# tamask1s/rspt

Measured on NVIDIA B200. Metric: compress_raw_GBps, higher is better.
Workload: dtype u8

## Files before the change

### include/rspt_gpu.h

```cpp
#ifndef RSPT_GPU_H_
#define RSPT_GPU_H_

#include <stddef.h>
#include <stdint.h>

#ifdef __cplusplus
extern "C" {
#endif

#define RSPT_GPU_ABI_VERSION 1

enum {
    RSPT_XDELTA_HZR = 0,
    RSPT_HZR = 1,
    RSPT_HADAMARD = 2,
    RSPT_DCT = 3
};

enum {
    RSPT_OK = 0,
    RSPT_E_ARG = -1,
    RSPT_E_CUDA = -2,
    RSPT_E_CAPACITY = -3,
    RSPT_E_STREAM = -4,
// ... 57 lines not shown
int rspt_gpu_sync(rspt_gpu_packer* p);
const char* rspt_gpu_last_error(const rspt_gpu_packer* p);

typedef struct {
    uint64_t frames_compressed, frames_decompressed;
    uint64_t raw_bytes_in, compressed_bytes_out;
    uint64_t blocks_copy, blocks_huff, blocks_fill;
    uint64_t escalations;
    uint64_t crc_failures;
    uint64_t kernel_launches;
} rspt_gpu_counters;
int rspt_gpu_get_counters(rspt_gpu_packer* p, rspt_gpu_counters* out);

enum {
    RSPT_STAGE_TRANSFORM = 0,
    RSPT_STAGE_HIST = 1,
    RSPT_STAGE_TREE = 2,
    RSPT_STAGE_LAYOUT = 3,
    RSPT_STAGE_ENCODE = 4,
    RSPT_STAGE_PARSE = 5,
    RSPT_STAGE_DECODE = 6,
    RSPT_STAGE_INVERSE = 7,
    RSPT_STAGE_COUNT = 8
};
int rspt_gpu_set_stage_timing(rspt_gpu_packer* p, int enable);
int rspt_gpu_get_stage_times(rspt_gpu_packer* p, double* ms ,
                             uint64_t* calls , int reset);

int rspt_gpu_debug_planes(rspt_gpu_packer* p, const uint8_t* d_src, size_t n_frames,
                          uint8_t* d_planes , uint8_t* d_header );
int rspt_gpu_debug_hzr_tables(rspt_gpu_packer* p, const uint8_t* d_block, size_t n,
                              uint32_t* d_hist , uint32_t* d_codes ,
                              uint32_t* d_info );
int rspt_gpu_crc32c(const uint8_t* d_data, size_t n, uint32_t* h_crc, void* stream);

int rspt_gpu_synth_ecg(uint8_t* d_dst, uint64_t first_frame, size_t n_frames, int bps, int ch, int ns,
                       uint64_t seed, int32_t amplitude, int32_t sigma, void* stream);

int rspt_gpu_prdn_terms(const uint8_t* d_orig, const uint8_t* d_dec, size_t n_frames, int bps, int ch,
                        int ns, double* h_out, void* stream);

int rspt_gpu_comm_unique_id(uint8_t id[128]);
int rspt_gpu_comm_init(int world, const uint8_t id[128], int rank, int device, void** comm);
int rspt_gpu_comm_destroy(void* comm);

int rspt_gpu_allgather_totals(void* comm, const uint64_t* d_total, uint64_t* d_all_totals, void* stream);

int rspt_gpu_rebase_offsets(uint64_t* d_offsets, size_t n_frames_plus_1, const uint64_t* d_all_totals,
                            int rank, void* stream);

int rspt_gpu_place_offsets_async(rspt_gpu_packer* p, void* comm, uint64_t* d_offsets, size_t n_frames, int rank, int world);
int rspt_gpu_place_join(rspt_gpu_packer* p);

int rspt_gpu_set_stream(rspt_gpu_packer* p, void* stream);

int rspt_gpu_set_dct_exact(rspt_gpu_packer* p, int exact);

#ifdef __cplusplus
}
#endif
#endif
```

### rspt_b200/_lib.py

```python
from __future__ import annotations

import ctypes as C
import os

HERE = os.path.dirname(os.path.abspath(__file__))
LIB_PATH = os.path.join(HERE, "librspt_gpu.so")

KINDS = {"xdelta_hzr": 0, "hzr": 1, "hadamard": 2, "dct": 3}
STAGES = ["transform", "hist", "tree", "layout", "encode", "parse", "decode", "inverse"]
ERRORS = {0: "ok", -1: "bad argument / unsupported shape", -2: "CUDA error", -3: "capacity too small",
          -4: "malformed stream", -5: "no CUDA device", -6: "CRC-32C mismatch"}

EXPORTS = [
    "rspt_gpu_create", "rspt_gpu_destroy", "rspt_gpu_frame_bytes", "rspt_gpu_header_bytes",
    "rspt_gpu_max_compressed_size", "rspt_gpu_nb", "rspt_gpu_compress_batch", "rspt_gpu_decompress_batch",
    "rspt_gpu_sidecar_bytes", "rspt_gpu_sidecar_used_bytes", "rspt_gpu_compress_host", "rspt_gpu_decompress_host",
    "rspt_gpu_compress_batch_host", "rspt_gpu_decompress_batch_host", "rspt_gpu_sync", "rspt_gpu_last_error",
    "rspt_gpu_get_counters", "rspt_gpu_debug_planes", "rspt_gpu_debug_hzr_tables", "rspt_gpu_crc32c",
    "rspt_gpu_synth_ecg", "rspt_gpu_prdn_terms", "rspt_gpu_rebase_offsets",
    "rspt_gpu_set_stage_timing", "rspt_gpu_get_stage_times", "rspt_gpu_verify_batch", "rspt_gpu_build_index",
    "rspt_gpu_prefilter_iir", "rspt_gpu_prefilter_fir",
    "rspt_gpu_ingest_create", "rspt_gpu_ingest_destroy", "rspt_gpu_ingest_next_address_to_fill", "rspt_gpu_ingest_drain",
    "rspt_gpu_comm_unique_id", "rspt_gpu_comm_init", "rspt_gpu_comm_destroy", "rspt_gpu_allgather_totals",
    "rspt_gpu_place_offsets_async", "rspt_gpu_place_join", "rspt_gpu_set_stream", "rspt_gpu_set_dct_exact",
]


class Counters(C.Structure):
    _fields_ = [(n, C.c_uint64) for n in (
        "frames_compressed", "frames_decompressed", "raw_bytes_in", "compressed_bytes_out",
        "blocks_copy", "blocks_huff", "blocks_fill", "escalations", "crc_failures", "kernel_launches")]


class RsptError(RuntimeError):
    pass


_lib = None


def lib() -> C.CDLL:
    global _lib
    if _lib is not None:
        return _lib
    if not os.path.exists(LIB_PATH):
        raise RsptError(f"{LIB_PATH} is missing: run `python -m rspt_b200.build` (nvcc, sm_100a). "
                        "There is no CPU fallback.")
    L = C.CDLL(LIB_PATH)
    sz, vp, u64 = C.c_size_t, C.c_void_p, C.c_uint64
    L.rspt_gpu_create.restype = C.c_int
    L.rspt_gpu_create.argtypes = [C.c_int, sz, sz, sz, sz, C.c_int, vp, sz, C.POINTER(vp)]
# ... 17 lines not shown
    L.rspt_gpu_prefilter_iir.argtypes = [vp, vp, sz, dp, dp, C.c_int, C.c_int]
    L.rspt_gpu_prefilter_fir.restype = C.c_int
    L.rspt_gpu_prefilter_fir.argtypes = [vp, vp, sz, dp, C.c_int]
    L.rspt_gpu_ingest_create.restype = C.c_int
    L.rspt_gpu_ingest_create.argtypes = [vp, sz, C.POINTER(vp)]
    L.rspt_gpu_ingest_destroy.restype = C.c_int
    L.rspt_gpu_ingest_destroy.argtypes = [vp]
    L.rspt_gpu_ingest_next_address_to_fill.restype = vp
    L.rspt_gpu_ingest_next_address_to_fill.argtypes = [vp]
    L.rspt_gpu_ingest_drain.restype = C.c_int
    L.rspt_gpu_ingest_drain.argtypes = [vp, C.c_int, vp, sz, vp, C.POINTER(sz)]
    L.rspt_gpu_build_index.restype = C.c_int
    L.rspt_gpu_build_index.argtypes = [vp, vp, vp, sz, vp, vp, vp]
    L.rspt_gpu_verify_batch.restype = C.c_int
    L.rspt_gpu_verify_batch.argtypes = [vp, vp, vp, sz, vp, vp]
    L.rspt_gpu_compress_host.restype = C.c_int
    L.rspt_gpu_compress_host.argtypes = [vp, vp, vp, sz, C.POINTER(sz)]
    L.rspt_gpu_decompress_host.restype = C.c_int
    L.rspt_gpu_decompress_host.argtypes = [vp, vp, C.POINTER(sz), vp]
    L.rspt_gpu_compress_batch_host.restype = C.c_int
    L.rspt_gpu_compress_batch_host.argtypes = [vp, vp, sz, vp, sz, vp]
    L.rspt_gpu_decompress_batch_host.restype = C.c_int
    L.rspt_gpu_decompress_batch_host.argtypes = [vp, vp, vp, sz, vp]
    L.rspt_gpu_sync.restype = C.c_int
    L.rspt_gpu_sync.argtypes = [vp]
    L.rspt_gpu_last_error.restype = C.c_char_p
    L.rspt_gpu_last_error.argtypes = [vp]
    L.rspt_gpu_get_counters.restype = C.c_int
    L.rspt_gpu_get_counters.argtypes = [vp, C.POINTER(Counters)]
    L.rspt_gpu_debug_planes.restype = C.c_int
    L.rspt_gpu_debug_planes.argtypes = [vp, vp, sz, vp, vp]
    L.rspt_gpu_debug_hzr_tables.restype = C.c_int
    L.rspt_gpu_debug_hzr_tables.argtypes = [vp, vp, sz, vp, vp, vp]
    L.rspt_gpu_crc32c.restype = C.c_int
    L.rspt_gpu_crc32c.argtypes = [vp, sz, C.POINTER(C.c_uint32), vp]
    L.rspt_gpu_synth_ecg.restype = C.c_int
    L.rspt_gpu_synth_ecg.argtypes = [vp, u64, sz, C.c_int, C.c_int, C.c_int, u64, C.c_int32, C.c_int32, vp]
    L.rspt_gpu_prdn_terms.restype = C.c_int
    L.rspt_gpu_prdn_terms.argtypes = [vp, vp, sz, C.c_int, C.c_int, C.c_int, C.POINTER(C.c_double), vp]
    L.rspt_gpu_rebase_offsets.restype = C.c_int
    L.rspt_gpu_rebase_offsets.argtypes = [vp, sz, vp, C.c_int, vp]
    L.rspt_gpu_set_stage_timing.restype = C.c_int
    L.rspt_gpu_set_stage_timing.argtypes = [vp, C.c_int]
    L.rspt_gpu_get_stage_times.restype = C.c_int
    L.rspt_gpu_get_stage_times.argtypes = [vp, C.POINTER(C.c_double), C.POINTER(u64), C.c_int]
    L.rspt_gpu_comm_unique_id.restype = C.c_int
    L.rspt_gpu_comm_unique_id.argtypes = [vp]
    L.rspt_gpu_comm_init.restype = C.c_int
    L.rspt_gpu_comm_init.argtypes = [C.c_int, vp, C.c_int, C.c_int, C.POINTER(vp)]
    L.rspt_gpu_comm_destroy.restype = C.c_int
    L.rspt_gpu_comm_destroy.argtypes = [vp]
    L.rspt_gpu_allgather_totals.restype = C.c_int
    L.rspt_gpu_allgather_totals.argtypes = [vp, vp, vp, vp]
    L.rspt_gpu_place_offsets_async.restype = C.c_int
    L.rspt_gpu_place_offsets_async.argtypes = [vp, vp, vp, sz, C.c_int, C.c_int]
    L.rspt_gpu_place_join.restype = C.c_int
    L.rspt_gpu_place_join.argtypes = [vp]
    L.rspt_gpu_set_stream.restype = C.c_int
    L.rspt_gpu_set_stream.argtypes = [vp, vp]
    L.rspt_gpu_set_dct_exact.restype = C.c_int
    L.rspt_gpu_set_dct_exact.argtypes = [vp, C.c_int]
    _lib = L
    return L


def check(rc: int, handle=None, what: str = "") -> None:
# ... 9 lines not shown
```

### rspt_b200/csrc/hzr_tree.cuh

```cuda
#pragma once

#include "common.cuh"

namespace rspt {

constexpr int kTreeWarps = 2;

struct TreeWarpSmem {
    uint32_t key[264];
    uint32_t icnt[260];
    uint32_t child[260];
    uint32_t ninfo[260];
    uint32_t tree[kTreeWords];
    uint16_t front[2][264];
    uint32_t pad;
};

struct Counters {
    unsigned long long frames_compressed, frames_decompressed, raw_bytes_in, compressed_bytes_out;
    unsigned long long blocks_copy, blocks_huff, blocks_fill, escalations;
    unsigned long long crc_failures;
};

__device__ __forceinline__ void blk_decode(const Shape& s, uint32_t blk, uint32_t& f, uint32_t& k, uint32_t& b)
{
    b = blk % s.nblk;
    uint32_t fk = blk / s.nblk;
    k = fk % s.nb_alloc;
    f = fk / s.nb_alloc;
}

__device__ __forceinline__ const uint8_t* blk_ptr(const uint8_t* planes, const Shape& s, uint32_t f, uint32_t k, uint32_t b)
{
    return planes + ((size_t)f * s.nb_alloc + k) * s.plane_stride + (size_t)b * kBlock;
}


__device__ __forceinline__ bool tree_prepare(TreeWarpSmem& S, const uint32_t* h, uint32_t* codes_out, uint32_t& L_out, BlkInfo& bi)
{
    const uint32_t lane = lane_id();
    uint32_t L = 0, nz = 0, nzsym = 0, zero_class = 0;
    uint32_t mykey = 0xFFFFFFFFu;
#pragma unroll
    for (int r = 0; r < 9; ++r) {
        const uint32_t sym = r * 32 + lane;
        const uint32_t c = sym < kNumSymbols ? h[sym] : 0u;
        const bool used = c != 0;
        const uint32_t m = __ballot_sync(0xFFFFFFFFu, used);
        const uint32_t pos = L + __popc(m & ((1u << lane) - 1u));
// ... 100 lines not shown
        id = take_int ? 512u + fr : li;
        wt = take_int ? ic : lc;
        lv = take_int ? ch >> 20 : 1u;
        if (take_int) {
            ic = nfr < ni ? raw & kInf : kInf;
            icf = nfr < ni ? raw & kEqNext : 0u;
        } else {
            lc = nli < L ? nk >> 9 : kInf;
        }
        fr = nfr;
        li = nli;
    };
    for (uint32_t round = 0; round + 1 < L; ++round) {
        uint32_t id0, id1, w0, w1, lv0, lv1;
        pick(id0, w0, lv0);
        pick(id1, w1, lv1);
        const uint32_t w = w0 + w1;
        if (w == last_w) {
            S.icnt[ni - 1] = w | kEqNext;
            if (ni - 1 == fr) icf = kEqNext;
        }
        if (fr == ni) {
            ic = w;
            icf = 0;
        }
        S.icnt[ni] = w;
        S.child[ni] = id0 | (id1 << 10) | ((lv0 + lv1) << 20);
        last_w = w;
        ++ni;
    }
    S.icnt[L - 2] = 0;
    S.ninfo[L - 2] = 0;
    S.front[0][0] = (uint16_t)(L - 2);
}

__device__ __forceinline__ BlkInfo tree_assign(TreeWarpSmem& S, const uint32_t L, uint32_t n, uint32_t* codes_out, uint32_t* tree_out)
{
    const uint32_t lane = lane_id();
    BlkInfo bi;
    uint32_t token_bits = 0, maxlen = 0, ntok = 0;
    {
        auto leaf = [&](uint32_t rank, uint32_t code, uint32_t depth, uint32_t off) {
            const uint32_t kv = S.key[rank];
            const uint32_t sym = 511u - (kv & 511u), cnt = kv >> 9;
            codes_out[sym] = code | (depth << 27);
            token_bits += cnt * (depth + sym_extra_bits(sym));
            ntok += cnt;
            maxlen = max(maxlen, depth);
            const unsigned long long bits = (unsigned long long)(1u | (sym << 1)) << (off & 31u);
            atomicOr(&S.tree[off >> 5], (uint32_t)bits);
            if (bits >> 32) atomicOr(&S.tree[(off >> 5) + 1], (uint32_t)(bits >> 32));
        };
        uint32_t nf = 1, cur = 0;
        const uint32_t lt = (1u << lane) - 1u;
        while (nf) {
            uint32_t nn = 0;
            for (uint32_t fb = 0; fb < nf; fb += 32) {
                const uint32_t i = fb + lane;
                const bool act = i < nf;
                uint32_t a = 0, bb = 0;
                if (act) {
                    const uint32_t j = S.front[cur][i];
                    const uint32_t ch = S.child[j], code = S.icnt[j], inf = S.ninfo[j];
                    const uint32_t depth = inf & 255u, off = inf >> 8;
                    a = ch & 1023u;
                    bb = (ch >> 10) & 1023u;
// ... 17 lines not shown
                const uint32_t ma = __ballot_sync(0xFFFFFFFFu, ia), mb = __ballot_sync(0xFFFFFFFFu, ib);
                if (ia) S.front[cur ^ 1][nn + __popc(ma & lt)] = (uint16_t)(a - 512u);
                nn += __popc(ma);
                if (ib) S.front[cur ^ 1][nn + __popc(mb & lt)] = (uint16_t)(bb - 512u);
                nn += __popc(mb);
            }
            __syncwarp();
            cur ^= 1;
            nf = nn;
        }
    }
#pragma unroll
    for (int o = 16; o > 0; o >>= 1) {
        token_bits += __shfl_xor_sync(0xFFFFFFFFu, token_bits, o);
        ntok += __shfl_xor_sync(0xFFFFFFFFu, ntok, o);
        maxlen = max(maxlen, __shfl_xor_sync(0xFFFFFFFFu, maxlen, o));
    }
    __syncwarp();
    const uint32_t tree_nbits = 11u * L - 1u;
    for (uint32_t i = lane; i < ((tree_nbits + 31u) >> 5); i += 32) tree_out[i] = S.tree[i];
    bi.tree_nbits = (uint16_t)tree_nbits;
    bi.total_bits = tree_nbits + token_bits;
    const uint32_t bytes = (bi.total_bits + 7u) >> 3;
    const bool copy = bytes > n || bytes >= kBlock || maxlen > 27u;
    bi.mode = copy ? MODE_COPY : MODE_HUFF;
    bi.payload_len = copy ? n : bytes;
    bi.fill = (uint8_t)maxlen;
    bi.n_used = (uint16_t)L;
    bi.n_tokens = (uint16_t)min(ntok, 65535u);
    return bi;
}

__device__ __forceinline__ BlkInfo warp_build_tree(TreeWarpSmem& S, const uint32_t* h, uint32_t n,
                                                   uint32_t* codes_out, uint32_t* tree_out)
{
    BlkInfo bi;
    uint32_t L;
    if (tree_prepare(S, h, codes_out, L, bi)) return bi;
    if (lane_id() == 0) tree_merge(S, L);
    __syncwarp();
    return tree_assign(S, L, n, codes_out, tree_out);
}

__device__ __forceinline__ void count_block_mode(Counters* ctr, uint32_t mode)
{
    atomicAdd(mode == MODE_FILL ? &ctr->blocks_fill : (mode == MODE_COPY ? &ctr->blocks_copy : &ctr->blocks_huff), 1ull);
}

__device__ __forceinline__ void warp_hist_from_list(const uint32_t* __restrict__ list, uint32_t m, uint32_t n, uint32_t* h)
{
    for (uint32_t i = lane_id(); i <= m; i += 32) {
        const uint32_t rs = i ? (list[i - 1] & 0xFFFFu) + 1u : 0u;
        uint32_t cur = n;
        if (i < m) {
            const uint32_t e = list[i];
            cur = e & 0xFFFFu;
            atomicAdd(&h[e >> 16], 1u);
        }
        uint32_t z = cur > rs ? cur - rs : 0u;
        while (z > kRunCap) {
            atomicAdd(&h[260], 1u);
            z -= kRunCap;
        }
        if (z) {
            const uint32_t idx = (z >= 2u) + (z >= 3u) + (z >= 7u) + (z >= 23u) + (z >= 279u);
            atomicAdd(&h[idx ? 255u + idx : 0u], 1u);
        }
    }
}

__global__ void __launch_bounds__(kTreeWarps * 32) k_hzr_tree(const uint32_t* __restrict__ hist, Shape s,
                                                               const uint8_t* __restrict__ frame_nb,
                                                               const uint8_t* __restrict__ blk_class, uint32_t cls,
                                                               uint32_t total_blocks,
                                                               uint32_t* __restrict__ codes,
                                                               uint32_t* __restrict__ tree,
                                                               BlkInfo* __restrict__ info,
                                                               Counters* __restrict__ ctr,
                                                               const uint32_t* __restrict__ list_n = nullptr, uint32_t sparse_stage = 0,
                                                               uint8_t* __restrict__ redo = nullptr,
                                                               const uint32_t* __restrict__ sub_n = nullptr,
                                                               const uint8_t* __restrict__ planes = nullptr,
                                                               uint32_t* __restrict__ lists = nullptr, uint32_t list_cap = 0)
{
    __shared__ TreeWarpSmem s_all[kTreeWarps];
    TreeWarpSmem& S = s_all[warp_id()];
    const uint32_t blk = blockIdx.x * kTreeWarps + warp_id();
    if (blk >= total_blocks) return;
    uint32_t f, k, b;
    blk_decode(s, blk, f, k, b);
    if (k >= frame_nb[f] || (blk_class && blk_class[blk] != cls)) return;
    const uint32_t n = blk_len(s, b);
    const uint32_t* h = hist + (size_t)blk * kSymStride;
    if (sub_n && list_n[blk] != kNoList) {
        const uint32_t lane = lane_id();
        const uint32_t ns = (uint32_t)s.ns, c0 = (b * kBlock) / ns, c1 = (b * kBlock + n) / ns;
        uint32_t* dst = lists + (size_t)blk * list_cap;
        uint32_t at = 0;
        for (uint32_t c = c0; c < c1; ++c) {
            const uint32_t nc = sub_n[((size_t)f * s.nb_alloc + k) * s.ch + c];
            const uint32_t* sub = reinterpret_cast<const uint32_t*>(planes + ((size_t)f * s.nb_alloc + k) * s.plane_stride + (size_t)c * ns);
            for (uint32_t i = lane; i < nc; i += 32) dst[at + i] = sub[i];
            at += nc;
        }
        uint32_t* list_hist = S.ninfo;
        static_assert(kTreeWords >= 4, "the histogram of a listed block spans ninfo[260] and tree[0..3]");
        for (uint32_t i = lane; i < (uint32_t)kSymStride; i += 32) list_hist[i] = 0;
        __syncwarp();
        warp_hist_from_list(dst, at, n, list_hist);
        __syncwarp();
        h = list_hist;
    }
    const BlkInfo bi = warp_build_tree(S, h, n, codes + (size_t)blk * kSymStride, tree + (size_t)blk * kTreeWords);
    if (lane_id() == 0) {
        info[blk] = bi;
        count_block_mode(ctr, bi.mode);
        if (redo && bi.mode != MODE_FILL && list_n[blk] != kNoList && !sparse_block_is_packed_from_list(list_n[blk], bi, sparse_stage))
            redo[f] = 1;
    }
}

__global__ void __launch_bounds__(1024) k_hzr_tree_ls(const uint32_t* __restrict__ hist, Shape s,
                                                      const uint8_t* __restrict__ frame_nb,
                                                      const uint8_t* __restrict__ blk_class, uint32_t cls,
                                                      uint32_t total_blocks,
                                                      uint32_t* __restrict__ codes,
                                                      uint32_t* __restrict__ tree,
                                                      BlkInfo* __restrict__ info,
                                                      Counters* __restrict__ ctr)
{
    extern __shared__ __align__(16) uint8_t s_tree_raw[];
    TreeWarpSmem* s_all = reinterpret_cast<TreeWarpSmem*>(s_tree_raw);
    __shared__ uint32_t s_L[32];
    const uint32_t W = blockDim.x >> 5, wid = warp_id(), lane = lane_id();
    TreeWarpSmem& S = s_all[wid];
    const uint32_t blk = blockIdx.x * W + wid;
    uint32_t f = 0, k = 0, b = 0, n = 0, L = 0;
    bool live = blk < total_blocks, merge = false;
    BlkInfo bi;
    if (live) {
        blk_decode(s, blk, f, k, b);
        live = k < frame_nb[f] && !(blk_class && blk_class[blk] != cls);
    }
    if (live) {
        n = blk_len(s, b);
        merge = !tree_prepare(S, hist + (size_t)blk * kSymStride, codes + (size_t)blk * kSymStride, L, bi);
// ... 14 lines not shown
```

### rspt_b200/csrc/packer.cuh

```cuda
#pragma once

#include <cuda_runtime.h>
#include <stdint.h>
#include <stdio.h>
#include <string.h>

#include <vector>

#include "common.cuh"
#include "hzr_encode.cuh"

struct HostPipe {
    cudaStream_t s_in, s_out;
    cudaEvent_t ev_in[2], ev_comp[2], ev_off[2], ev_out[2];
    uint8_t* d_src[2];
    uint8_t* d_dst[2];
    uint64_t* d_off[2];
    uint64_t* h_off[2];
    size_t chunk;
};

struct rspt_gpu_packer {
    rspt::Shape s;
    int device;
// ... 23 lines not shown
    uint64_t* d_all_totals;
    uint16_t* d_step_lz;
    rspt::BlkInfo* d_info;
    uint8_t* d_frame_nb;
    uint32_t* d_need;
    uint32_t* d_nb_state;
    uint32_t* d_sizes;
    uint32_t* d_blk_off;
    uint8_t* d_headers;
    int32_t* d_words;
    long long* d_sums;
    rspt::Counters* d_ctr;
    const rspt::CrcConst* d_crc;
    void* d_dec;
    uint8_t* d_dec_nb;
    int32_t* d_status_tmp;
    uint8_t* d_seg_xor;
    uint32_t segs_per_plane;
    void* d_auto_index;
    uint32_t* d_inv_tot;
    uint32_t* d_inv_flag;
    uint32_t inv_epoch;
    double* d_fir;
    size_t fir_cap;
    int32_t* d_words2;
    uint8_t* d_redo;
    uint8_t* d_redo2;
    uint32_t* d_sub_n;
    bool front_ok;
    int front_grid;
    size_t front_smem;
    uint32_t sp_stage;
    bool sparse_list;
    double2* d_twiddle;
    double2* d_post;
    float* d_cos;
    uint8_t* d_one_src;
    uint8_t* d_one_dst;
    uint64_t* d_one_off;
    uint8_t* h_pin;
    size_t h_pin_bytes;
    uint8_t* d_hb_src;
    uint8_t* d_hb_dst;
    uint64_t* d_hb_off;
    size_t hb_frames;
    HostPipe pipe;

    unsigned long long launches;
    bool timing;
    std::vector<cudaEvent_t>* ev_free;
    struct Pending { int stage; cudaEvent_t a, b; };
    std::vector<Pending>* ev_pending;
    double stage_ms[8];
    unsigned long long stage_calls[8];
    char err[256];
};

namespace rspt {

inline int fail_cuda(rspt_gpu_packer* p, cudaError_t e, const char* what)
{
    if (p) snprintf(p->err, sizeof(p->err), "CUDA error %d (%s) at %s", (int)e, cudaGetErrorString(e), what);
    return -2;
}

inline int fail_arg(rspt_gpu_packer* p, const char* what)
// ... 7 lines not shown
```

### rspt_b200/csrc/rspt_gpu.cu

```cuda
#include "../../include/rspt_gpu.h"
#include "../../include/rspt_synth.h"

#include <dlfcn.h>
#include <stdlib.h>

#include <atomic>
#include <mutex>
#include <new>
#include <vector>

#include "packer.cuh"
#include "transforms.cuh"
#include "front.cuh"
#include "hzr_decode.cuh"
#include "spectral.cuh"
#include "filters.cuh"

using namespace rspt;

namespace {

constexpr int kMaxDevices = 64;
std::mutex g_mu;
CrcConst* g_crc[kMaxDevices] = {};
// ... 368 lines not shown
    if (e == cudaSuccess && kind == RSPT_DCT) e = dct_build_tables(p);
    const size_t maxc = rspt_gpu_max_compressed_size(p);
    A(dalloc(p->d_one_src, (size_t)s.frame_bytes));
    A(dalloc(p->d_one_dst, maxc));
    A(dalloc(p->d_one_off, 2));
    p->h_pin_bytes = maxc > s.frame_bytes ? maxc : s.frame_bytes;
    p->h_pin_bytes += 64;
    if (e == cudaSuccess) e = cudaMallocHost(reinterpret_cast<void**>(&p->h_pin), p->h_pin_bytes);
    if (e == cudaSuccess) e = cudaMemsetAsync(p->d_frame_nb, (int)s.nb_init, F, p->stream);
    if (e == cudaSuccess) e = cudaMemsetAsync(p->d_ctr, 0, sizeof(Counters), p->stream);
    if (e == cudaSuccess) e = cudaMemcpyAsync(p->d_nb_state, &s.nb_init, 4, cudaMemcpyHostToDevice, p->stream);
    if (e == cudaSuccess) e = allow_smem(k_hzr_encode<2>, kEncodeSmem);
    if (e == cudaSuccess) e = allow_smem(k_hzr_encode<3>, kEncodeSmem);
    if (e == cudaSuccess) e = allow_smem(k_hzr_hist<1>, kHistSmem);
    if (e == cudaSuccess) e = allow_smem(k_hzr_hist<3>, kHistSmemList);
    if (e == cudaSuccess) e = cudaStreamCreateWithFlags(&p->side, cudaStreamNonBlocking);
    if (e == cudaSuccess) e = cudaStreamCreateWithFlags(&p->place, cudaStreamNonBlocking);
    if (e == cudaSuccess) e = cudaEventCreateWithFlags(&p->ev_place, cudaEventDisableTiming);
    for (int k = 0; k < rspt_gpu_packer::kPlaceRing && e == cudaSuccess; ++k)
        e = cudaEventCreateWithFlags(&p->ev_placed[k], cudaEventDisableTiming);
    if (e == cudaSuccess) e = cudaEventCreateWithFlags(&p->ev_fork, cudaEventDisableTiming);
    if (e == cudaSuccess) e = cudaEventCreateWithFlags(&p->ev_join, cudaEventDisableTiming);
    if (e == cudaSuccess) e = cudaEventCreateWithFlags(&p->ev_fork2, cudaEventDisableTiming);
    if (e == cudaSuccess) e = cudaEventCreateWithFlags(&p->ev_join2, cudaEventDisableTiming);
    if (e == cudaSuccess) e = allow_smem(k_hzr_encode_sparse<true>, kSparseSmem);
    if (e == cudaSuccess) e = allow_smem(k_hzr_encode_sparse<false>, kSparseSmem);
    if (e == cudaSuccess) e = front_setup(p);
    {
        const char* ev = getenv("RSPT_SPARSE_STAGE_BYTES");
        const long v = ev ? atol(ev) : (long)kSpStageBytes;
        p->sp_stage = (uint32_t)(v < 1 ? 1 : (v > (long)kSpStageBytes ? (long)kSpStageBytes : v));
        const char* el = getenv("RSPT_SPARSE_LIST");
        p->sparse_list = !(el && atoi(el) == 0);
    }
    if (e == cudaSuccess) e = allow_smem(k_hzr_decode, kDecodeSmem);
    if (e == cudaSuccess) e = allow_smem(k_hzr_verify, kDecodeSmem);
    if (e == cudaSuccess) e = allow_smem(k_hzr_build_index, kDecodeSmem);
    if (e == cudaSuccess) e = allow_smem(k_crc32c, kEncodeSmem);
    if (e == cudaSuccess) e = cudaStreamSynchronize(p->stream);
    if (e != cudaSuccess) {
        fprintf(stderr, "rspt_gpu_create: %s\n", cudaGetErrorString(e));
        rspt_gpu_destroy(p);
        return RSPT_E_CUDA;
    }
    *out = p;
    return RSPT_OK;
}

extern "C" int rspt_gpu_destroy(rspt_gpu_packer* p)
{
    if (!p) return RSPT_E_ARG;
    DeviceGuard dg(p->device);
    cudaStreamSynchronize(p->stream);
    void* ptrs[] = {p->d_planes, p->d_hist, p->d_codes, p->d_tree, p->d_step_lz, p->d_lists, p->d_list_n, p->d_blk_class, p->d_info, p->d_frame_nb,
                    p->d_need, p->d_nb_state, p->d_sizes, p->d_blk_off, p->d_headers, p->d_words, p->d_sums, p->d_ctr,
                    p->d_dec, p->d_dec_nb, p->d_status_tmp, p->d_twiddle, p->d_post, p->d_cos, p->d_one_src, p->d_one_dst,
                    p->d_one_off, p->d_redo, p->d_redo2, p->d_sub_n, p->d_hb_src, p->d_hb_dst, p->d_hb_off, p->d_auto_index, p->d_fir, p->d_words2, p->d_inv_tot, p->d_inv_flag, p->d_all_totals, p->d_seg_xor};
    for (void* q : ptrs)
        if (q) cudaFree(q);
    if (p->h_pin) cudaFreeHost(p->h_pin);
    destroy_host_pipe(p);
    if (p->ev_pending) {
        ev_resolve(p);
        for (cudaEvent_t e : *p->ev_free) cudaEventDestroy(e);
        delete p->ev_pending;
        delete p->ev_free;
// ... 197 lines not shown
            RSPT_CUDA_CHECK(cudaStreamWaitEvent(p->stream, p->ev_placed[k], 0));
            p->placed_ptr[k] = nullptr;
        }
    return RSPT_OK;
}

extern "C" int rspt_gpu_compress_batch(rspt_gpu_packer* p, const uint8_t* d_src, size_t n_frames, uint8_t* d_dst,
                                       size_t dst_capacity, uint64_t* d_offsets, uint8_t* d_frame_nb, void* d_sidecar)
{
    if (!p || !d_src || !d_dst || !d_offsets) return RSPT_E_ARG;
    if (n_frames == 0) return RSPT_OK;
    if (n_frames > p->max_batch) return fail_arg(p, "n_frames exceeds max_batch_frames"), RSPT_E_CAPACITY;
    if (dst_capacity < n_frames * rspt_gpu_max_compressed_size(p))
        return fail_arg(p, "dst_capacity < n_frames * rspt_gpu_max_compressed_size"), RSPT_E_CAPACITY;
    DeviceGuard dg(p->device);
    const Shape& s = p->s;
    const size_t F = n_frames;
    const uint32_t nblocks = total_blocks(p, F);
    int rc = wait_for_placement_of(p, d_offsets);
    if (rc) return rc;
    uint32_t* sidecar = reinterpret_cast<uint32_t*>(d_sidecar);
    const unsigned tgrid = (nblocks + kTreeWarps - 1) / kTreeWarps;
    if (p->front_ok && !((uintptr_t)d_src & 15)) {
        {
            StageTimer t(p, RSPT_STAGE_TRANSFORM);
            front_launch(p, d_src, F, 0);
            front_launch(p, d_src, F, 1);
            p->launches += 2;
            RSPT_CUDA_CHECK(cudaGetLastError());
        }
        {
            StageTimer t(p, RSPT_STAGE_TREE);
            k_hzr_tree<<<tgrid, 32 * kTreeWarps, 0, p->stream>>>(p->d_hist, s, p->d_frame_nb, nullptr, 0, nblocks, p->d_codes, p->d_tree, p->d_info, p->d_ctr,
                                                                 p->d_list_n, p->sp_stage, p->d_redo2, p->d_sub_n, p->d_planes, p->d_lists, kListCap);
            front_launch(p, d_src, F, 2);
            p->launches += 2;
            RSPT_CUDA_CHECK(cudaGetLastError());
        }
    } else {
    {
        StageTimer t(p, RSPT_STAGE_TRANSFORM);
        rc = launch_forward_transform(p, d_src, F);
        if (rc) return rc;
        rc = launch_frame_nb(p, F);
        if (rc) return rc;
    }
    {
        RSPT_CUDA_CHECK(cudaEventRecord(p->ev_fork, p->stream));
        RSPT_CUDA_CHECK(cudaStreamWaitEvent(p->side, p->ev_fork, 0));
        launch_sparse_hist(p, p->d_planes, s, nblocks, p->side);
        if (const uint32_t W = tree_lockstep_warps())
            k_hzr_tree_ls<<<(nblocks + W - 1) / W, 32 * W, W * sizeof(TreeWarpSmem), p->side>>>(p->d_hist, s, p->d_frame_nb, p->d_blk_class, kClassSparse, nblocks, p->d_codes, p->d_tree, p->d_info, p->d_ctr);
        else
        k_hzr_tree<<<tgrid, 32 * kTreeWarps, 0, p->side>>>(p->d_hist, s, p->d_frame_nb, p->d_blk_class, kClassSparse, nblocks, p->d_codes, p->d_tree, p->d_info, p->d_ctr);
        RSPT_CUDA_CHECK(cudaEventRecord(p->ev_join, p->side));
        {
            StageTimer t(p, RSPT_STAGE_HIST);
            k_hzr_hist<2><<<nblocks, kHistThreads, 0, p->stream>>>(p->d_planes, s, p->d_frame_nb, p->d_hist, p->d_step_lz, p->d_lists, p->d_list_n, p->d_blk_class);
        }
        {
            StageTimer t(p, RSPT_STAGE_TREE);
            if (const uint32_t W = tree_lockstep_warps())
                k_hzr_tree_ls<<<(nblocks + W - 1) / W, 32 * W, W * sizeof(TreeWarpSmem), p->stream>>>(p->d_hist, s, p->d_frame_nb, p->d_blk_class, kClassDense, nblocks, p->d_codes, p->d_tree, p->d_info, p->d_ctr);
            else
            k_hzr_tree<<<tgrid, 32 * kTreeWarps, 0, p->stream>>>(p->d_hist, s, p->d_frame_nb, p->d_blk_class, kClassDense, nblocks, p->d_codes, p->d_tree, p->d_info, p->d_ctr);
            RSPT_CUDA_CHECK(cudaStreamWaitEvent(p->stream, p->ev_join, 0));
        }
        p->launches += 4;
    }
    }
    {
        StageTimer t(p, RSPT_STAGE_LAYOUT);
        k_frame_sizes<<<(unsigned)((F + 255) / 256), 256, 0, p->stream>>>(p->d_info, s, p->d_frame_nb, (uint32_t)F, p->d_sizes, p->d_blk_off);
        k_scan_offsets<<<1, 1024, 0, p->stream>>>(p->d_sizes, (uint32_t)F, d_offsets, p->d_ctr, s.frame_bytes);
    }
    {
        StageTimer t(p, RSPT_STAGE_ENCODE);
        const SparseOut so{d_dst, d_offsets, p->d_blk_off, p->sp_stage, p->d_headers, sidecar};
        RSPT_CUDA_CHECK(cudaEventRecord(p->ev_fork2, p->stream));
        RSPT_CUDA_CHECK(cudaStreamWaitEvent(p->side, p->ev_fork2, 0));
        if (p->sparse_list)
            k_hzr_encode_sparse<true><<<nblocks, kSpThreads, kSparseSmem, p->side>>>(s, p->d_frame_nb, p->d_info, p->d_codes, p->d_tree, p->d_lists,
                                                                                     p->d_list_n, p->d_crc, so);
        else
            k_hzr_encode_sparse<false><<<nblocks, kSpThreads, kSparseSmem, p->side>>>(s, p->d_frame_nb, p->d_info, p->d_codes, p->d_tree, p->d_lists,
                                                                                      p->d_list_n, p->d_crc, so);
        RSPT_CUDA_CHECK(cudaEventRecord(p->ev_join2, p->side));
        if (encode_ctas_per_sm(s) == 3)
            k_hzr_encode<3><<<nblocks, kEncThreads, p->enc_smem, p->stream>>>(p->d_planes, s, p->d_frame_nb, p->d_info, p->d_blk_off,
                                                                               p->d_codes, p->d_tree, p->d_step_lz, p->d_lists, p->d_list_n, p->sp_stage,
                                                                               d_offsets, p->d_headers, p->d_crc, d_dst, sidecar);
        else
            k_hzr_encode<2><<<nblocks, kEncThreads, p->enc_smem, p->stream>>>(p->d_planes, s, p->d_frame_nb, p->d_info, p->d_blk_off,
                                                                               p->d_codes, p->d_tree, p->d_step_lz, p->d_lists, p->d_list_n, p->sp_stage,
                                                                               d_offsets, p->d_headers, p->d_crc, d_dst, sidecar);
        RSPT_CUDA_CHECK(cudaStreamWaitEvent(p->stream, p->ev_join2, 0));
    }
    p->launches += 4;
// ... 652 lines not shown
        RSPT_CUDA_CHECK(cudaStreamWaitEvent(hp.s_out, hp.ev_comp[b], 0));
        RSPT_CUDA_CHECK(cudaMemcpyAsync(h_dst + f0 * fb, hp.d_src[b], nf * fb, cudaMemcpyDeviceToHost, hp.s_out));
        RSPT_CUDA_CHECK(cudaEventRecord(hp.ev_out[b], hp.s_out));
    }
    RSPT_CUDA_CHECK(cudaStreamSynchronize(hp.s_out));
    RSPT_CUDA_CHECK(cudaStreamSynchronize(p->stream));
    return RSPT_OK;
}

extern "C" int rspt_gpu_debug_planes(rspt_gpu_packer* p, const uint8_t* d_src, size_t n_frames, uint8_t* d_planes,
                                     uint8_t* d_header)
{
    if (!p || !d_src || !d_planes || n_frames > p->max_batch) return RSPT_E_ARG;
    DeviceGuard dg(p->device);
    int rc = launch_forward_transform(p, d_src, n_frames);
    if (rc) return rc;
    const Shape& s = p->s;
    RSPT_CUDA_CHECK(cudaMemcpy2DAsync(d_planes, s.N, p->d_planes, s.plane_stride, s.N, n_frames * s.nb_alloc,
                                      cudaMemcpyDeviceToDevice, p->stream));
    if (d_header && s.hdr_bytes)
        RSPT_CUDA_CHECK(cudaMemcpyAsync(d_header, p->d_headers, n_frames * s.hdr_bytes, cudaMemcpyDeviceToDevice, p->stream));
    return RSPT_OK;
}

extern "C" int rspt_gpu_debug_hzr_tables(rspt_gpu_packer* p, const uint8_t* d_block, size_t n, uint32_t* d_hist,
                                         uint32_t* d_codes, uint32_t* d_info)
{
    if (!p || !d_block || n < 1 || n > kBlock || ((uintptr_t)d_block & 15)) return RSPT_E_ARG;
    DeviceGuard dg(p->device);
    Shape s = p->s;
    s.N = (uint32_t)n; s.nblk = 1; s.nb_alloc = 1; s.plane_stride = (uint32_t)((n + 15) & ~(size_t)15);
    launch_sparse_hist(p, d_block, s, 1, p->stream);
    k_hzr_hist<2><<<1, kHistThreads, 0, p->stream>>>(d_block, s, p->d_frame_nb, p->d_hist, p->d_step_lz, p->d_lists, p->d_list_n, p->d_blk_class);
    k_hzr_tree<<<1, 32 * kTreeWarps, 0, p->stream>>>(p->d_hist, s, p->d_frame_nb, p->d_blk_class, kClassSparse, 1, p->d_codes, p->d_tree, p->d_info, p->d_ctr);
    k_hzr_tree<<<1, 32 * kTreeWarps, 0, p->stream>>>(p->d_hist, s, p->d_frame_nb, p->d_blk_class, kClassDense, 1, p->d_codes, p->d_tree, p->d_info, p->d_ctr);
    p->launches += 4;
    RSPT_CUDA_CHECK(cudaGetLastError());
    if (d_hist) RSPT_CUDA_CHECK(cudaMemcpyAsync(d_hist, p->d_hist, kNumSymbols * 4, cudaMemcpyDeviceToDevice, p->stream));
    if (d_codes) RSPT_CUDA_CHECK(cudaMemcpyAsync(d_codes, p->d_codes, kNumSymbols * 4, cudaMemcpyDeviceToDevice, p->stream));
    if (d_info) {
        RSPT_CUDA_CHECK(cudaStreamSynchronize(p->stream));
        BlkInfo bi;
        RSPT_CUDA_CHECK(cudaMemcpy(&bi, p->d_info, sizeof(bi), cudaMemcpyDeviceToHost));
        uint32_t v[4] = {bi.mode, bi.payload_len, bi.tree_nbits, bi.n_used};
        RSPT_CUDA_CHECK(cudaMemcpy(d_info, v, sizeof(v), cudaMemcpyHostToDevice));
    }
    return RSPT_OK;
}

extern "C" int rspt_gpu_crc32c(const uint8_t* d_data, size_t n, uint32_t* h_crc, void* stream)
{
    if (!d_data || !h_crc || n > kBlock) return RSPT_E_ARG;
    int dev = 0;
    if (cudaGetDevice(&dev) != cudaSuccess) return RSPT_E_NOGPU;
    int rc = ensure_device_constants(dev);
    if (rc) return rc;
    uint32_t* d_out = static_cast<uint32_t*>(result_slot(dev));
    allow_smem(k_crc32c, kEncodeSmem);
    k_crc32c<<<1, 1024, kEncodeSmem, (cudaStream_t)stream>>>(d_data, (uint32_t)n, g_crc[dev], 3, d_out);
    cudaError_t e = cudaMemcpyAsync(h_crc, d_out, 4, cudaMemcpyDeviceToHost, (cudaStream_t)stream);
    if (e == cudaSuccess) e = cudaStreamSynchronize((cudaStream_t)stream);
    return e == cudaSuccess ? RSPT_OK : RSPT_E_CUDA;
}

namespace {

template <int BPS>
__global__ void __launch_bounds__(256) k_synth(uint8_t* __restrict__ dst, uint64_t first, uint32_t n_frames, int ch, int ns,
                                               rspt_synth_params prm, const int32_t* __restrict__ tab)
{
    const uint32_t tiles = ((uint32_t)ns + 255u) / 256u;
    const uint32_t f = blockIdx.x / tiles, s = (blockIdx.x % tiles) * 256u + threadIdx.x;
    if (f >= n_frames || s >= (uint32_t)ns) return;
    const int32_t* beat = tab;
    const int32_t* sine = tab + RSPT_SYNTH_TABLE;
    uint8_t* out = dst + ((size_t)f * ns + s) * ch * BPS;
    for (int c = 0; c < ch; ++c) {
        const rspt_synth_chan k = rspt_synth_channel(&prm, first + f, (uint32_t)c);
        const uint32_t v = (uint32_t)rspt_synth_sample(&prm, &k, beat, sine, first + f, (uint32_t)c, s, BPS);
// ... 114 lines not shown
```

### rspt_b200/packer.py

```python
from __future__ import annotations

import ctypes as C
from dataclasses import dataclass

import numpy as np
import torch

from . import _lib
from ._lib import KINDS, Counters, RsptError, check


@dataclass
class CompressedBatch:
    stream: torch.Tensor
    offsets: torch.Tensor
    frame_nb: torch.Tensor
    sidecar: torch.Tensor | None
    n_frames: int

    def total_bytes(self) -> int:
        return int(self.offsets[-1].item())

    def frame(self, i: int) -> bytes:
        off = self.offsets[i:i + 2].cpu().tolist()
# ... 211 lines not shown
        rc = self.L.rspt_gpu_compress_batch_host(self.h, frames.ctypes.data, n, dst.ctypes.data, dst.size, offsets.ctypes.data)
        check(rc, self.h, "rspt_gpu_compress_batch_host")
        return int(offsets[n])

    def decompress_batch_host(self, src: np.ndarray, offsets: np.ndarray, out: np.ndarray) -> None:
        n = offsets.size - 1
        rc = self.L.rspt_gpu_decompress_batch_host(self.h, src.ctypes.data, offsets.ctypes.data, n, out.ctypes.data)
        check(rc, self.h, "rspt_gpu_decompress_batch_host")

    def debug_planes(self, frames: torch.Tensor):
        n = frames.numel() // self.frame_bytes
        unsigned = C.c_uint(0)
        nb_alloc = (self.max_compressed_size - 1 - self.header_bytes) // (4 + 4 + 7 * ((self.ch * self.ns + 65535) // 65536) + self.ch * self.ns)
        planes = torch.empty(n * nb_alloc * self.ch * self.ns, dtype=torch.uint8, device=self._dev())
        hdr = torch.zeros(max(1, n * self.header_bytes), dtype=torch.uint8, device=self._dev())
        check(self.L.rspt_gpu_debug_planes(self.h, frames.data_ptr(), n, planes.data_ptr(), hdr.data_ptr()), self.h, "debug_planes")
        torch.cuda.synchronize(self._dev())
        return planes.cpu().numpy().reshape(n, nb_alloc, self.ch * self.ns), hdr.cpu().numpy()[: n * self.header_bytes].reshape(n, -1)

    def debug_hzr_tables(self, block: np.ndarray):
        dev = self._dev()
        b = torch.from_numpy(np.ascontiguousarray(block, np.uint8)).to(dev)
        pad = torch.zeros(64, dtype=torch.uint8, device=dev)
        b = torch.cat([b, pad])
        hist = torch.zeros(264, dtype=torch.int32, device=dev)
        codes = torch.zeros(264, dtype=torch.int32, device=dev)
        info = torch.zeros(4, dtype=torch.int32, device=dev)
        check(self.L.rspt_gpu_debug_hzr_tables(self.h, b.data_ptr(), block.size, hist.data_ptr(), codes.data_ptr(), info.data_ptr()),
              self.h, "debug_hzr_tables")
        torch.cuda.synchronize(dev)
        return (hist.cpu().numpy().view(np.uint32)[:261], codes.cpu().numpy().view(np.uint32)[:261],
                info.cpu().numpy().view(np.uint32))


class IngestRing:

    def __init__(self, packer: SignalPacker, nr_max_packets: int):
        self.p = packer
        self.L = packer.L
        self.h = C.c_void_p()
        check(self.L.rspt_gpu_ingest_create(packer.h, nr_max_packets, C.byref(self.h)), packer.h, "rspt_gpu_ingest_create")

    def close(self):
        if self.h:
            self.L.rspt_gpu_ingest_destroy(self.h)
            self.h = C.c_void_p()

    def next_packet(self):
        addr = self.L.rspt_gpu_ingest_next_address_to_fill(self.h)
        if not addr:
            return None
        return np.ctypeslib.as_array(C.cast(addr, C.POINTER(C.c_uint8)), shape=(self.p.frame_bytes,))

    def drain(self, dst: np.ndarray, offsets: np.ndarray, max_frames: int | None = None, flush: bool = False) -> int:
        n = C.c_size_t(offsets.size - 1 if max_frames is None else min(max_frames, offsets.size - 1))
        rc = self.L.rspt_gpu_ingest_drain(self.h, int(flush), dst.ctypes.data, dst.size, offsets.ctypes.data, C.byref(n))
        check(rc, self.p.h, "rspt_gpu_ingest_drain")
        return int(n.value)


def crc32c(data: np.ndarray) -> int:
    t = torch.from_numpy(np.array(data, dtype=np.uint8, copy=True)).cuda() if data.size else torch.zeros(1, dtype=torch.uint8, device="cuda")
    out = C.c_uint32(0)
    check(_lib.lib().rspt_gpu_crc32c(t.data_ptr(), data.size, C.byref(out), torch.cuda.current_stream().cuda_stream), None, "crc32c")
    return out.value

# ... 22 lines not shown
```

Baseline: 557.1.

## Add warp-parallel phased Huffman tree merge for large alphabets

Adds a warp-cooperative Huffman merge. Each phase uses ballots to count the leaves and internal nodes below a threshold weight, places the merged items by rank with binary search, and forms parent pairs in parallel. It replaces the single-lane sequential merge when the symbol count is at least 33, which is the default and can be changed through an environment variable. The aim is to cut serial latency in the tree-build stage, at the cost of more complex code, extra shared-memory traffic, and correctness risk on tie ordering. A debug entry point for testing trees on given histograms is also added.

```diff
diff --git a/include/rspt_gpu.h b/include/rspt_gpu.h
--- a/include/rspt_gpu.h
+++ b/include/rspt_gpu.h
@@ -113,6 +113,10 @@
 int rspt_gpu_debug_hzr_tables(rspt_gpu_packer* p, const uint8_t* d_block, size_t n,
                               uint32_t* d_hist , uint32_t* d_codes ,
                               uint32_t* d_info );
+int rspt_gpu_debug_hzr_trees(rspt_gpu_packer* p, const uint32_t* d_hist, size_t n_hist,
+                             uint32_t* d_codes ,
+                             uint32_t* d_tree ,
+                             uint32_t* d_info );
 int rspt_gpu_crc32c(const uint8_t* d_data, size_t n, uint32_t* h_crc, void* stream);
 
 int rspt_gpu_synth_ecg(uint8_t* d_dst, uint64_t first_frame, size_t n_frames, int bps, int ch, int ns,
diff --git a/rspt_b200/_lib.py b/rspt_b200/_lib.py
--- a/rspt_b200/_lib.py
+++ b/rspt_b200/_lib.py
@@ -16,7 +16,8 @@
     "rspt_gpu_max_compressed_size", "rspt_gpu_nb", "rspt_gpu_compress_batch", "rspt_gpu_decompress_batch",
     "rspt_gpu_sidecar_bytes", "rspt_gpu_sidecar_used_bytes", "rspt_gpu_compress_host", "rspt_gpu_decompress_host",
     "rspt_gpu_compress_batch_host", "rspt_gpu_decompress_batch_host", "rspt_gpu_sync", "rspt_gpu_last_error",
-    "rspt_gpu_get_counters", "rspt_gpu_debug_planes", "rspt_gpu_debug_hzr_tables", "rspt_gpu_crc32c",
+    "rspt_gpu_get_counters", "rspt_gpu_debug_planes", "rspt_gpu_debug_hzr_tables", "rspt_gpu_debug_hzr_trees",
+    "rspt_gpu_crc32c",
     "rspt_gpu_synth_ecg", "rspt_gpu_prdn_terms", "rspt_gpu_rebase_offsets",
     "rspt_gpu_set_stage_timing", "rspt_gpu_get_stage_times", "rspt_gpu_verify_batch", "rspt_gpu_build_index",
     "rspt_gpu_prefilter_iir", "rspt_gpu_prefilter_fir",
@@ -100,6 +101,8 @@
     L.rspt_gpu_debug_planes.argtypes = [vp, vp, sz, vp, vp]
     L.rspt_gpu_debug_hzr_tables.restype = C.c_int
     L.rspt_gpu_debug_hzr_tables.argtypes = [vp, vp, sz, vp, vp, vp]
+    L.rspt_gpu_debug_hzr_trees.restype = C.c_int
+    L.rspt_gpu_debug_hzr_trees.argtypes = [vp, vp, sz, vp, vp, vp]
     L.rspt_gpu_crc32c.restype = C.c_int
     L.rspt_gpu_crc32c.argtypes = [vp, sz, C.POINTER(C.c_uint32), vp]
     L.rspt_gpu_synth_ecg.restype = C.c_int
diff --git a/rspt_b200/csrc/hzr_tree.cuh b/rspt_b200/csrc/hzr_tree.cuh
--- a/rspt_b200/csrc/hzr_tree.cuh
+++ b/rspt_b200/csrc/hzr_tree.cuh
@@ -1,10 +1,13 @@
 #pragma once
 
+#include <cstddef>
+
 #include "common.cuh"
 
 namespace rspt {
 
 constexpr int kTreeWarps = 2;
+constexpr uint32_t kPhasedMinL = 33;
 
 struct TreeWarpSmem {
     uint32_t key[264];
@@ -15,6 +18,8 @@
     uint16_t front[2][264];
     uint32_t pad;
 };
+
+static_assert(offsetof(TreeWarpSmem, front) % 4 == 0, "TreeWarpSmem::front must be 4-byte aligned");
 
 struct Counters {
     unsigned long long frames_compressed, frames_decompressed, raw_bytes_in, compressed_bytes_out;
@@ -181,6 +186,76 @@
     S.icnt[L - 2] = 0;
     S.ninfo[L - 2] = 0;
     S.front[0][0] = (uint16_t)(L - 2);
+}
+
+__device__ __forceinline__ uint32_t count_lt(const uint32_t* a, uint32_t n, uint32_t x)
+{
+    uint32_t pos = 0;
+    for (uint32_t step = n ? 1u << (31 - __clz(n)) : 0u; step; step >>= 1)
+        pos += (pos + step <= n && a[pos + step - 1] < x) ? step : 0u;
+    return pos;
+}
+
+__device__ __forceinline__ void tree_merge_phased(TreeWarpSmem& S, const uint32_t L)
+{
+    constexpr uint32_t kInf = 0x7FFFFFFFu, kNone = 0xFFFFFFFFu;
+    const uint32_t lane = lane_id();
+    uint16_t* const item = S.front[0];
+    uint32_t li = 0, fr = 0, ni = 0;
+    uint32_t cid = kNone, cw = 0;
+    while ((L - li) + (ni - fr) + (cid != kNone ? 1u : 0u) > 1u) {
+        const uint32_t l0 = li < L ? S.key[li] >> 9 : kInf, l1 = li + 1u < L ? S.key[li + 1u] >> 9 : kInf;
+        const uint32_t i0 = fr < ni ? S.icnt[fr] : kInf, i1 = fr + 1u < ni ? S.icnt[fr + 1u] : kInf;
+        const uint32_t h0 = min(l0, i0);
+        const uint32_t t = cid != kNone ? cw + h0 : h0 + min(max(l0, i0), min(l1, i1));
+        const uint32_t tk = t << 9;
+        uint32_t nl, nint;
+        {
+            const uint32_t a = li + 9u * lane + 8u, b = fr + 9u * lane + 8u;
+            const uint32_t cl = 9u * __popc(__ballot_sync(0xFFFFFFFFu, a < L && S.key[a] < tk));
+            const uint32_t ci = 9u * __popc(__ballot_sync(0xFFFFFFFFu, b < ni && S.icnt[b] < t));
+            const uint32_t a2 = li + cl + lane, b2 = fr + ci + lane;
+            nl = cl + __popc(__ballot_sync(0xFFFFFFFFu, lane < 9u && a2 < L && S.key[a2] < tk));
+            nint = ci + __popc(__ballot_sync(0xFFFFFFFFu, lane < 9u && b2 < ni && S.icnt[b2] < t));
+        }
+        const uint32_t c = cid != kNone ? 1u : 0u, m = c + nl + nint;
+        const uint32_t* const lk = S.key + li;
+        const uint32_t* const iw = S.icnt + fr;
+        if (c && lane == 0) item[0] = (uint16_t)cid;
+        for (uint32_t p = lane; p < nl; p += 32) {
+            const uint32_t w = lk[p] >> 9;
+            item[c + p + count_lt(iw, nint, w + 1u)] = (uint16_t)(li + p);
+        }
+        for (uint32_t q = lane; q < nint; q += 32) {
+            const uint32_t w = iw[q];
+            const uint32_t r = count_lt(iw, nint, w) + count_lt(iw, nint, w + 1u) - 1u - q + count_lt(lk, nl, w << 9);
+            item[c + r] = (uint16_t)(512u + fr + q);
+        }
+        __syncwarp();
+        auto weight = [&](uint32_t x) { return x < 512u ? S.key[x] >> 9 : S.icnt[x - 512u]; };
+        auto leaves = [&](uint32_t x) { return x < 512u ? 1u : S.child[x - 512u] >> 20; };
+        const uint32_t* const pairs = reinterpret_cast<const uint32_t*>(item);
+        for (uint32_t q = lane; q < (m >> 1); q += 32) {
+            const uint32_t ab = pairs[q], a = ab & 0xFFFFu, b = ab >> 16;
+            S.icnt[ni + q] = weight(a) + weight(b);
+            S.child[ni + q] = a | (b << 10) | ((leaves(a) + leaves(b)) << 20);
+        }
+        if (m & 1u) {
+            cid = item[m - 1u];
+            cw = weight(cid);
+        } else {
+            cid = kNone;
+        }
+        li += nl;
+        fr += nint;
+        ni += m >> 1;
+        __syncwarp();
+    }
+    if (lane == 0) {
+        S.icnt[L - 2] = 0;
+        S.ninfo[L - 2] = 0;
+        S.front[0][0] = (uint16_t)(L - 2);
+    }
 }
 
 __device__ __forceinline__ BlkInfo tree_assign(TreeWarpSmem& S, const uint32_t L, uint32_t n, uint32_t* codes_out, uint32_t* tree_out)
@@ -264,12 +339,13 @@
 }
 
 __device__ __forceinline__ BlkInfo warp_build_tree(TreeWarpSmem& S, const uint32_t* h, uint32_t n,
-                                                   uint32_t* codes_out, uint32_t* tree_out)
+                                                   uint32_t* codes_out, uint32_t* tree_out, uint32_t phased_min)
 {
     BlkInfo bi;
     uint32_t L;
     if (tree_prepare(S, h, codes_out, L, bi)) return bi;
-    if (lane_id() == 0) tree_merge(S, L);
+    if (L >= phased_min) tree_merge_phased(S, L);
+    else if (lane_id() == 0) tree_merge(S, L);
     __syncwarp();
     return tree_assign(S, L, n, codes_out, tree_out);
 }
@@ -308,7 +384,7 @@
                                                                uint32_t* __restrict__ codes,
                                                                uint32_t* __restrict__ tree,
                                                                BlkInfo* __restrict__ info,
-                                                               Counters* __restrict__ ctr,
+                                                               Counters* __restrict__ ctr, uint32_t phased_min,
                                                                const uint32_t* __restrict__ list_n = nullptr, uint32_t sparse_stage = 0,
                                                                uint8_t* __restrict__ redo = nullptr,
                                                                const uint32_t* __restrict__ sub_n = nullptr,
@@ -343,7 +419,8 @@
         __syncwarp();
         h = list_hist;
     }
-    const BlkInfo bi = warp_build_tree(S, h, n, codes + (size_t)blk * kSymStride, tree + (size_t)blk * kTreeWords);
+    const BlkInfo bi = warp_build_tree(S, h, n, codes + (size_t)blk * kSymStride, tree + (size_t)blk * kTreeWords,
+                                     phased_min);
     if (lane_id() == 0) {
         info[blk] = bi;
         count_block_mode(ctr, bi.mode);
diff --git a/rspt_b200/csrc/packer.cuh b/rspt_b200/csrc/packer.cuh
--- a/rspt_b200/csrc/packer.cuh
+++ b/rspt_b200/csrc/packer.cuh
@@ -79,6 +79,7 @@
     size_t front_smem;
     uint32_t sp_stage;
     bool sparse_list;
+    uint32_t tree_phased_min;
     double2* d_twiddle;
     double2* d_post;
     float* d_cos;
diff --git a/rspt_b200/csrc/rspt_gpu.cu b/rspt_b200/csrc/rspt_gpu.cu
--- a/rspt_b200/csrc/rspt_gpu.cu
+++ b/rspt_b200/csrc/rspt_gpu.cu
@@ -424,6 +424,9 @@
         p->sp_stage = (uint32_t)(v < 1 ? 1 : (v > (long)kSpStageBytes ? (long)kSpStageBytes : v));
         const char* el = getenv("RSPT_SPARSE_LIST");
         p->sparse_list = !(el && atoi(el) == 0);
+        const char* em = getenv("RSPT_TREE_MERGE");
+        const int tm = em ? atoi(em) : 1;
+        p->tree_phased_min = tm == 0 ? 0xFFFFFFFFu : (tm == 2 ? 2u : kPhasedMinL);
     }
     if (e == cudaSuccess) e = allow_smem(k_hzr_decode, kDecodeSmem);
     if (e == cudaSuccess) e = allow_smem(k_hzr_verify, kDecodeSmem);
@@ -687,7 +690,7 @@
         {
             StageTimer t(p, RSPT_STAGE_TREE);
             k_hzr_tree<<<tgrid, 32 * kTreeWarps, 0, p->stream>>>(p->d_hist, s, p->d_frame_nb, nullptr, 0, nblocks, p->d_codes, p->d_tree, p->d_info, p->d_ctr,
-                                                                 p->d_list_n, p->sp_stage, p->d_redo2, p->d_sub_n, p->d_planes, p->d_lists, kListCap);
+                                                                 p->tree_phased_min, p->d_list_n, p->sp_stage, p->d_redo2, p->d_sub_n, p->d_planes, p->d_lists, kListCap);
             front_launch(p, d_src, F, 2);
             p->launches += 2;
             RSPT_CUDA_CHECK(cudaGetLastError());
@@ -707,7 +710,7 @@
         if (const uint32_t W = tree_lockstep_warps())
             k_hzr_tree_ls<<<(nblocks + W - 1) / W, 32 * W, W * sizeof(TreeWarpSmem), p->side>>>(p->d_hist, s, p->d_frame_nb, p->d_blk_class, kClassSparse, nblocks, p->d_codes, p->d_tree, p->d_info, p->d_ctr);
         else
-        k_hzr_tree<<<tgrid, 32 * kTreeWarps, 0, p->side>>>(p->d_hist, s, p->d_frame_nb, p->d_blk_class, kClassSparse, nblocks, p->d_codes, p->d_tree, p->d_info, p->d_ctr);
+        k_hzr_tree<<<tgrid, 32 * kTreeWarps, 0, p->side>>>(p->d_hist, s, p->d_frame_nb, p->d_blk_class, kClassSparse, nblocks, p->d_codes, p->d_tree, p->d_info, p->d_ctr, p->tree_phased_min);
         RSPT_CUDA_CHECK(cudaEventRecord(p->ev_join, p->side));
         {
             StageTimer t(p, RSPT_STAGE_HIST);
@@ -718,7 +721,7 @@
             if (const uint32_t W = tree_lockstep_warps())
                 k_hzr_tree_ls<<<(nblocks + W - 1) / W, 32 * W, W * sizeof(TreeWarpSmem), p->stream>>>(p->d_hist, s, p->d_frame_nb, p->d_blk_class, kClassDense, nblocks, p->d_codes, p->d_tree, p->d_info, p->d_ctr);
             else
-            k_hzr_tree<<<tgrid, 32 * kTreeWarps, 0, p->stream>>>(p->d_hist, s, p->d_frame_nb, p->d_blk_class, kClassDense, nblocks, p->d_codes, p->d_tree, p->d_info, p->d_ctr);
+            k_hzr_tree<<<tgrid, 32 * kTreeWarps, 0, p->stream>>>(p->d_hist, s, p->d_frame_nb, p->d_blk_class, kClassDense, nblocks, p->d_codes, p->d_tree, p->d_info, p->d_ctr, p->tree_phased_min);
             RSPT_CUDA_CHECK(cudaStreamWaitEvent(p->stream, p->ev_join, 0));
         }
         p->launches += 4;
@@ -1437,8 +1440,8 @@
     s.N = (uint32_t)n; s.nblk = 1; s.nb_alloc = 1; s.plane_stride = (uint32_t)((n + 15) & ~(size_t)15);
     launch_sparse_hist(p, d_block, s, 1, p->stream);
     k_hzr_hist<2><<<1, kHistThreads, 0, p->stream>>>(d_block, s, p->d_frame_nb, p->d_hist, p->d_step_lz, p->d_lists, p->d_list_n, p->d_blk_class);
-    k_hzr_tree<<<1, 32 * kTreeWarps, 0, p->stream>>>(p->d_hist, s, p->d_frame_nb, p->d_blk_class, kClassSparse, 1, p->d_codes, p->d_tree, p->d_info, p->d_ctr);
-    k_hzr_tree<<<1, 32 * kTreeWarps, 0, p->stream>>>(p->d_hist, s, p->d_frame_nb, p->d_blk_class, kClassDense, 1, p->d_codes, p->d_tree, p->d_info, p->d_ctr);
+    k_hzr_tree<<<1, 32 * kTreeWarps, 0, p->stream>>>(p->d_hist, s, p->d_frame_nb, p->d_blk_class, kClassSparse, 1, p->d_codes, p->d_tree, p->d_info, p->d_ctr, p->tree_phased_min);
+    k_hzr_tree<<<1, 32 * kTreeWarps, 0, p->stream>>>(p->d_hist, s, p->d_frame_nb, p->d_blk_class, kClassDense, 1, p->d_codes, p->d_tree, p->d_info, p->d_ctr, p->tree_phased_min);
     p->launches += 4;
     RSPT_CUDA_CHECK(cudaGetLastError());
     if (d_hist) RSPT_CUDA_CHECK(cudaMemcpyAsync(d_hist, p->d_hist, kNumSymbols * 4, cudaMemcpyDeviceToDevice, p->stream));
@@ -1450,6 +1453,39 @@
         uint32_t v[4] = {bi.mode, bi.payload_len, bi.tree_nbits, bi.n_used};
         RSPT_CUDA_CHECK(cudaMemcpy(d_info, v, sizeof(v), cudaMemcpyHostToDevice));
     }
+    return RSPT_OK;
+}
+
+extern "C" int rspt_gpu_debug_hzr_trees(rspt_gpu_packer* p, const uint32_t* d_hist, size_t n_hist, uint32_t* d_codes,
+                                        uint32_t* d_tree, uint32_t* d_info)
+{
+    if (!p || !d_hist || !d_codes || !d_tree || !d_info || n_hist < 1 || n_hist > 65535) return RSPT_E_ARG;
+    DeviceGuard dg(p->device);
+    Shape s = p->s;
+    s.nblk = (uint32_t)n_hist; s.nb_alloc = 1; s.N = (uint32_t)n_hist * kBlock;
+    const size_t ctr_off = n_hist * sizeof(BlkInfo), nb_off = ctr_off + sizeof(Counters);
+    uint8_t* d_scratch = nullptr;
+    RSPT_CUDA_CHECK(cudaMalloc(&d_scratch, nb_off + 1));
+    BlkInfo* d_bi = reinterpret_cast<BlkInfo*>(d_scratch);
+    cudaError_t e = cudaMemsetAsync(d_scratch, 0, nb_off, p->stream);
+    if (e == cudaSuccess) e = cudaMemsetAsync(d_scratch + nb_off, 1, 1, p->stream);
+    if (e == cudaSuccess) {
+        k_hzr_tree<<<(unsigned)((n_hist + kTreeWarps - 1) / kTreeWarps), 32 * kTreeWarps, 0, p->stream>>>(
+            d_hist, s, d_scratch + nb_off, nullptr, 0, (uint32_t)n_hist, d_codes, d_tree, d_bi,
+            reinterpret_cast<Counters*>(d_scratch + ctr_off), p->tree_phased_min);
+        p->launches += 1;
+        e = cudaGetLastError();
+    }
+    std::vector<BlkInfo> bi(n_hist);
+    if (e == cudaSuccess) e = cudaMemcpyAsync(bi.data(), d_bi, n_hist * sizeof(BlkInfo), cudaMemcpyDeviceToHost, p->stream);
+    if (e == cudaSuccess) e = cudaStreamSynchronize(p->stream);
+    cudaFree(d_scratch);
+    RSPT_CUDA_CHECK(e);
+    std::vector<uint32_t> v(4 * n_hist);
+    for (size_t i = 0; i < n_hist; ++i) {
+        v[4 * i] = bi[i].mode; v[4 * i + 1] = bi[i].payload_len; v[4 * i + 2] = bi[i].tree_nbits; v[4 * i + 3] = bi[i].n_used;
+    }
+    RSPT_CUDA_CHECK(cudaMemcpy(d_info, v.data(), v.size() * 4, cudaMemcpyHostToDevice));
     return RSPT_OK;
 }
 
diff --git a/rspt_b200/packer.py b/rspt_b200/packer.py
--- a/rspt_b200/packer.py
+++ b/rspt_b200/packer.py
@@ -267,6 +267,22 @@
         return (hist.cpu().numpy().view(np.uint32)[:261], codes.cpu().numpy().view(np.uint32)[:261],
                 info.cpu().numpy().view(np.uint32))
 
+    def debug_hzr_trees(self, hists: np.ndarray):
+        dev = self._dev()
+        hists = np.asarray(hists, np.uint32)
+        n = hists.shape[0]
+        h = np.zeros((n, 264), np.uint32)
+        h[:, :hists.shape[1]] = hists
+        d_hist = torch.from_numpy(h.view(np.int32)).to(dev)
+        codes = torch.zeros((n, 264), dtype=torch.int32, device=dev)
+        tree = torch.zeros((n, 92), dtype=torch.int32, device=dev)
+        info = torch.zeros((n, 4), dtype=torch.int32, device=dev)
+        check(self.L.rspt_gpu_debug_hzr_trees(self.h, d_hist.data_ptr(), n, codes.data_ptr(), tree.data_ptr(), info.data_ptr()),
+              self.h, "debug_hzr_trees")
+        torch.cuda.synchronize(dev)
+        return (codes.cpu().numpy().view(np.uint32)[:, :261], tree.cpu().numpy().view(np.uint8),
+                info.cpu().numpy().view(np.uint32))
+
 
 class IngestRing:
 
```

New measurement: 589.3, median of 6. 5.8% higher.
